# ideafisher/ssUnet-GAN

Hardware: AMD Instinct MI355X
Metric: train images/sec (512^2 tiles) (higher is better)
Workload: dtype f32; 1 GPU; UNet_R_SS_v2 generator + SRGAN-style discriminator, one G+D step (train_seg_gan.py:182-233), 16 x 3x512x512 tiles per GPU, fp32, Adam lr 2e-5; global_batch=16, tile=512, parallelism=dp1, dead_d_param_grads_of_g_step=computed

## Files before the change

ssunet-gan_amd/csrc/conv_wgrad4.hip:

```cpp
#include "common.h"
#include "conv_thin.h"
#include <type_traits>

namespace {

struct W4Args {
  const float* wide; const float* thin; float* ws;
  int Cw, ldw, ldt, N, H, W, Cout, Cin, Cin_real;
  int groups, nz;
  long long units_per_z;
  int segs_per_row;
};

constexpr int SEG = 32;
constexpr int U = 8;

template <bool THIN_COUT, int KS>
__global__ __launch_bounds__(256) void wgrad4_kernel(const W4Args a) {
  constexpr int R = KS / 2, NT = KS * KS, COLS = U + KS - 1;
  const int lane = threadIdx.x & 63;
  const int wave = threadIdx.x >> 6;
  const int zb = blockIdx.x / a.groups, cg = blockIdx.x - zb * a.groups;
  const int z = zb * 4 + wave;
  const int j = lane & 3;
  const int cw = cg * 64 + lane;
  const bool cw_ok = cw < a.Cw;
  const float* tapT = THIN_COUT ? a.wide : a.thin;
  const float* fixT = THIN_COUT ? a.thin : a.wide;
  const unsigned ldtap = THIN_COUT ? a.ldw : a.ldt, ldfix = THIN_COUT ? a.ldt : a.ldw;
  const unsigned npix = (unsigned)(a.N * a.H * a.W);
  const auto tap_rs = __builtin_amdgcn_make_buffer_rsrc(const_cast<float*>(tapT), 0, (int)(npix * ldtap * 4u), 0x00020000);
  const auto fix_rs = __builtin_amdgcn_make_buffer_rsrc(const_cast<float*>(fixT), 0, (int)(npix * ldfix * 4u), 0x00020000);
  const unsigned chtap = THIN_COUT ? cw : j, chfix = THIN_COUT ? j : cw;
  const bool tap_lane_ok = THIN_COUT ? cw_ok : true, fix_lane_ok = THIN_COUT ? true : cw_ok;
  constexpr unsigned OOB = 0xffffffffu;

  f32x4 acc[NT];
#pragma unroll
  for (int t = 0; t < NT; ++t) acc[t] = f32x4{0.f, 0.f, 0.f, 0.f};

  const int u0 = z * (int)a.units_per_z;
  const int total_units = a.N * a.H * a.segs_per_row;
  int u1 = u0 + (int)a.units_per_z; if (u1 > total_units) u1 = total_units;
  for (int u = u0; u < u1; ++u) {
    const int r = u / a.segs_per_row; const int seg = u - r * a.segs_per_row;
    const int y = r % a.H, n = r / a.H;
    const int x0 = seg * SEG;
    const int x1 = x0 + SEG < a.W ? x0 + SEG : a.W;
    unsigned rowoff[KS]; bool rowok[KS];
#pragma unroll
    for (int q = 0; q < KS; ++q) {
      const int iy = y + q - R;
      rowok[q] = tap_lane_ok && (unsigned)iy < (unsigned)a.H;
      rowoff[q] = ((unsigned)((n * a.H + iy) * a.W) * ldtap + chtap) * 4u;
    }
    const unsigned fixoff = ((unsigned)((n * a.H + y) * a.W) * ldfix + chfix) * 4u;
    for (int xb = x0; xb < x1; xb += U) {
      float f[U], v[KS][COLS];
#pragma unroll
      for (int k = 0; k < U; ++k) {
        const bool ok = fix_lane_ok && (xb + k < x1);
        f[k] = __builtin_bit_cast(float, __builtin_amdgcn_raw_buffer_load_b32(
            fix_rs, ok ? fixoff + (unsigned)(xb + k) * ldfix * 4u : OOB, 0, 0));
      }
#pragma unroll
      for (int c = 0; c < COLS; ++c) {
        const int ix = xb + c - R;
        const bool cok = (unsigned)ix < (unsigned)a.W;
        const unsigned xo = (unsigned)ix * ldtap * 4u;
#pragma unroll
        for (int q = 0; q < KS; ++q)
          v[q][c] = __builtin_bit_cast(float, __builtin_amdgcn_raw_buffer_load_b32(
              tap_rs, (cok && rowok[q]) ? rowoff[q] + xo : OOB, 0, 0));
      }
#pragma unroll
      for (int k = 0; k < U; ++k)
#pragma unroll
        for (int q = 0; q < KS; ++q)
#pragma unroll
          for (int e = 0; e < KS; ++e) {
            if (THIN_COUT) acc[q * KS + e] = __builtin_amdgcn_mfma_f32_4x4x1f32(v[q][k + e], f[k], acc[q * KS + e], 0, 0, 0);
            else acc[q * KS + e] = __builtin_amdgcn_mfma_f32_4x4x1f32(f[k], v[q][k + e], acc[q * KS + e], 0, 0, 0);
          }
    }
  }
  __shared__ float red[4][NT * 4][64];
#pragma unroll
  for (int t = 0; t < NT; ++t)
#pragma unroll
    for (int i = 0; i < 4; ++i) red[wave][t * 4 + i][lane] = acc[t][i];
  __syncthreads();
  float* slab = a.ws + (size_t)zb * NT * a.Cin * a.Cout;
  const int b4 = (lane >> 2) * 4;
  for (int e = wave; e < NT * 4; e += 4) {
    const int t = e >> 2, i = e & 3;
    const float sum = ((red[0][e][lane] + red[1][e][lane]) + red[2][e][lane]) + red[3][e][lane];
    int co, c;
    if (THIN_COUT) { co = j; c = cg * 64 + b4 + i; }
    else { co = cg * 64 + b4 + i; c = j; }
    if (co < a.Cout && c < a.Cin) slab[((size_t)t * a.Cin + c) * a.Cout + co] = sum;
  }
}

template <int CR>
__device__ __forceinline__ void wgrad32_cin_body(const W4Args& a, float (*red)[36][64]) {
  const int lane = threadIdx.x & 63, l31 = lane & 31, h = lane >> 5;
  const int wave = threadIdx.x >> 6;
  const int zb = blockIdx.x / a.groups, cg = blockIdx.x - zb * a.groups;
  const int z = zb * 4 + wave;
  const unsigned npix = (unsigned)(a.N * a.H * a.W);
  const auto do_rs = __builtin_amdgcn_make_buffer_rsrc(const_cast<float*>(a.wide), 0, (int)(npix * (unsigned)a.ldw * 4u), 0x00020000);
  const auto in_rs = __builtin_amdgcn_make_buffer_rsrc(const_cast<float*>(a.thin), 0, (int)(npix * (unsigned)a.ldt * 4u), 0x00020000);
  constexpr unsigned OOB = 0xffffffffu;
  const unsigned ldwb = (unsigned)a.ldw * 4u, ldtb = (unsigned)a.ldt * 4u;
  constexpr int NC = CR == 3 ? 27 : 32;
  unsigned aoff[2];
#pragma unroll
  for (int f = 0; f < 2; ++f) { const int co = cg * 64 + f * 32 + l31; aoff[f] = co < a.Cout ? (unsigned)co * 4u : OOB; }
  const int t0 = l31 / CR, c = l31 - t0 * CR;
  const int dy0 = t0 / 3 - 1, dx0 = t0 % 3 - 1;
  const bool col_ok = l31 < NC;

  f32x16 acc[2];
  f32x4 acc8[2];
#pragma unroll
  for (int f = 0; f < 2; ++f) {
#pragma unroll
    for (int q = 0; q < 16; ++q) acc[f][q] = 0.f;
    acc8[f] = f32x4{0.f, 0.f, 0.f, 0.f};
  }

  const int u0 = z * (int)a.units_per_z;
  const int total_units = a.N * a.H * a.segs_per_row;
  int u1 = u0 + (int)a.units_per_z; if (u1 > total_units) u1 = total_units;
  constexpr int UP = 8;
  for (int u = u0; u < u1; ++u) {
    const int r = u / a.segs_per_row; const int seg = u - r * a.segs_per_row;
    const int y = r % a.H, n = r / a.H;
    const int x0 = seg * SEG;
    const int x1 = x0 + SEG < a.W ? x0 + SEG : a.W;
    const unsigned rowpix = (unsigned)((n * a.H + y) * a.W);
    const bool r0ok = col_ok && (unsigned)(y + dy0) < (unsigned)a.H, r8ok = y + 1 < a.H;
    const unsigned b0row = (rowpix + (unsigned)(dy0 * a.W)) * ldtb + (unsigned)c * 4u;
    const unsigned b8row = (rowpix + (unsigned)a.W) * ldtb + (unsigned)(lane & 3) * 4u;
    auto step = [&](auto full_c, const int xb) {
      constexpr bool FULL = decltype(full_c)::value;
      float av[2][UP], bv[UP], b8[UP];
#pragma unroll
      for (int k = 0; k < UP; ++k) {
        const int x = xb + 2 * k + h;
        const bool pok = FULL || x < x1;
        const unsigned po = (rowpix + (unsigned)x) * ldwb;
#pragma unroll
        for (int f = 0; f < 2; ++f)
          av[f][k] = __builtin_bit_cast(float, __builtin_amdgcn_raw_buffer_load_b32(do_rs, (pok && aoff[f] != OOB) ? po + aoff[f] : OOB, 0, 0));
        const int ix0 = x + dx0;
        bv[k] = __builtin_bit_cast(float, __builtin_amdgcn_raw_buffer_load_b32(
            in_rs, (pok && r0ok && (unsigned)ix0 < (unsigned)a.W) ? b0row + (unsigned)ix0 * ldtb : OOB, 0, 0));
        if (CR == 4)
          b8[k] = __builtin_bit_cast(float, __builtin_amdgcn_raw_buffer_load_b32(
              in_rs, (pok && r8ok && x + 1 < a.W) ? b8row + (unsigned)(x + 1) * ldtb : OOB, 0, 0));
      }
#pragma unroll
      for (int k = 0; k < UP; ++k)
#pragma unroll
        for (int f = 0; f < 2; ++f) {
          acc[f] = __builtin_amdgcn_mfma_f32_32x32x2f32(av[f][k], bv[k], acc[f], 0, 0, 0);
          if (CR == 4) acc8[f] = __builtin_amdgcn_mfma_f32_4x4x1f32(av[f][k], b8[k], acc8[f], 0, 0, 0);
        }
    };
    for (int xb = x0; xb < x1; xb += 2 * UP) {
      if (xb + 2 * UP <= x1) step(std::true_type{}, xb);
      else step(std::false_type{}, xb);
    }
  }
  if (col_ok) {
#pragma unroll
    for (int f = 0; f < 2; ++f)
#pragma unroll
      for (int q = 0; q < 16; ++q) red[wave][l31][f * 32 + (q & 3) + 8 * (q >> 2) + 4 * h] = acc[f][q];
  }
  if (CR == 4) {
#pragma unroll
    for (int f = 0; f < 2; ++f)
#pragma unroll
      for (int i = 0; i < 4; ++i) {
        const float odd = __shfl(acc8[f][i], l31 + 32);
        const float s8 = acc8[f][i] + odd;
        if (h == 0) red[wave][32 + (lane & 3)][f * 32 + (l31 & ~3) + i] = s8;
      }
  }
  __syncthreads();
  float* slab = a.ws + (size_t)zb * 9 * a.Cin * a.Cout;
  constexpr int NR = CR == 3 ? 27 : 36;
  for (int e = threadIdx.x; e < NR * 64; e += 256) {
    const int nn = e >> 6, m = e & 63;
    const float sum = ((red[0][nn][m] + red[1][nn][m]) + red[2][nn][m]) + red[3][nn][m];
    const int co = cg * 64 + m;
    const int row = CR == 3 ? nn + nn / 3 : nn;
    if (co < a.Cout) slab[(size_t)row * a.Cout + co] = sum;
  }
}

__global__ __launch_bounds__(256) void wgrad32_cin_kernel(const W4Args a) {
  __shared__ float red[4][36][64];
  if (a.Cin_real == 3) wgrad32_cin_body<3>(a, red);
  else wgrad32_cin_body<4>(a, red);
}

constexpr int TINY_PIX = 4096;

__global__ __launch_bounds__(256) void wgrad_tiny4_kernel(const W4Args a) {
  const int co = threadIdx.x & 7, slot = threadIdx.x >> 3;
  const long long npix = (long long)a.N * a.H * a.W;
  const long long p0 = (long long)blockIdx.x * TINY_PIX;
  const long long p1 = p0 + TINY_PIX < npix ? p0 + TINY_PIX : npix;
  const auto in_rs = __builtin_amdgcn_make_buffer_rsrc(const_cast<float*>(a.thin), 0, (int)((unsigned)npix * (unsigned)a.ldt * 4u), 0x00020000);
  const auto do_rs = __builtin_amdgcn_make_buffer_rsrc(const_cast<float*>(a.wide), 0, (int)((unsigned)npix * (unsigned)a.ldw * 4u), 0x00020000);
  constexpr unsigned OOB = 0xffffffffu;
  const bool co_ok = co < a.Cout;
  f32x4 acc[9];
#pragma unroll
  for (int t = 0; t < 9; ++t) acc[t] = f32x4{0.f, 0.f, 0.f, 0.f};
  for (long long p = p0 + slot; p < p1; p += 32) {
    const int x = (int)(p % a.W); const int y = (int)((p / a.W) % a.H);
    const float g = __builtin_bit_cast(float, __builtin_amdgcn_raw_buffer_load_b32(do_rs, co_ok ? ((unsigned)p * (unsigned)a.ldw + (unsigned)co) * 4u : OOB, 0, 0));
#pragma unroll
    for (int t = 0; t < 9; ++t) {
      const int iy = y + t / 3 - 1, ix = x + t % 3 - 1;
      const bool ok = (unsigned)iy < (unsigned)a.H && (unsigned)ix < (unsigned)a.W;
      const f32x4 v = __builtin_bit_cast(f32x4, __builtin_amdgcn_raw_buffer_load_b128(
          in_rs, ok ? (unsigned)(p + (long long)(t / 3 - 1) * a.W + (t % 3 - 1)) * (unsigned)a.ldt * 4u : OOB, 0, 0));
      acc[t] += v * g;
    }
  }
  __shared__ float red[32][36][8];
#pragma unroll
  for (int t = 0; t < 9; ++t)
#pragma unroll
    for (int c = 0; c < 4; ++c) red[slot][t * 4 + c][co] = acc[t][c];
  __syncthreads();
  float* slab = a.ws + (size_t)blockIdx.x * 9 * a.Cin * a.Cout;
  for (int e = threadIdx.x; e < 36 * 8; e += 256) {
    const int c8 = e & 7, row = e >> 3;
    float sum = 0.f;
#pragma unroll 8
    for (int k = 0; k < 32; ++k) sum += red[k][row][c8];
    const int t = row >> 2, c = row & 3;
    if (c8 < a.Cout && c < a.Cin) slab[((size_t)t * a.Cin + c) * a.Cout + c8] = sum;
  }
}

}

int ssg_wgrad4_kind(const ssg_wgrad_desc* d) {
  if (d->C2 != 0 || d->in_sy != 1 || d->in_sx != 1 || d->GH != d->H || d->GW != d->W) return 0;
  if (d->ntaps == 9) {
    for (int t = 0; t < 9; ++t) if (d->dy[t] != t / 3 - 1 || d->dx[t] != t % 3 - 1) return 0;
  } else if (d->ntaps != 1 || d->dy[0] != 0 || d->dx[0] != 0) {
    return 0;
  }
  if ((long long)d->N * d->H * d->W * (d->ld1 > d->ldd ? d->ld1 : d->ldd) >= (1ll << 30)) return 0;
  if (d->Cout <= 4 && d->C1 >= 16 && d->C1 % 4 == 0) return 5;
  if (d->C1 == 4 && d->Cout <= 8 && d->ntaps == 9) return 7;
  if (d->C1 == 4 && d->ntaps == 9 && d->Cout >= 32 && (long long)d->N * d->H * d->W >= 65536) return 8;
  if (d->C1 == 4) return 6;
  return 0;
}

int ssg_wgrad4_slices(const ssg_wgrad_desc* d, int kind, int* groups, long long* units_per_z, int* segs_per_row) {
  if (kind == 7) {
    if (groups) *groups = 1;
    if (units_per_z) *units_per_z = TINY_PIX;
    if (segs_per_row) *segs_per_row = 1;
    return (int)(((long long)d->N * d->H * d->W + TINY_PIX - 1) / TINY_PIX);
  }
  const int cw = kind == 5 ? d->C1 : d->Cout;
  const int g = (cw + 63) / 64;
  const int spr = (d->W + SEG - 1) / SEG;
  const long long units = (long long)d->N * d->H * spr;
  long long nz = 8192 / g;
  if (nz > units) nz = units;
  if (nz < 1) nz = 1;
  const long long upz = (units + nz - 1) / nz;
  nz = (units + upz - 1) / upz;
  nz = (nz + 3) / 4;
  if (groups) *groups = g;
  if (units_per_z) *units_per_z = upz;
  if (segs_per_row) *segs_per_row = spr;
  return (int)nz;
}

int ssg_wgrad4_launch(const ssg_wgrad_desc* d, int kind, hipStream_t st) {
  W4Args a;
  a.ws = d->ws; a.N = d->N; a.H = d->H; a.W = d->W; a.Cout = d->Cout; a.Cin = d->C1; a.Cin_real = d->Cin_real;
  a.nz = ssg_wgrad4_slices(d, kind, &a.groups, &a.units_per_z, &a.segs_per_row);
  const dim3 grid((unsigned)(a.nz * a.groups)), block(256);
  if (kind == 7) {
    a.wide = d->dout; a.Cw = d->Cout; a.ldw = d->ldd; a.thin = d->in1; a.ldt = d->ld1;
    hipLaunchKernelGGL(wgrad_tiny4_kernel, grid, block, 0, st, a);
    SSG_LAUNCH_CHECK();
    return SSG_OK;
  }
  if (kind == 8) {
    a.wide = d->dout; a.Cw = d->Cout; a.ldw = d->ldd; a.thin = d->in1; a.ldt = d->ld1;
    hipLaunchKernelGGL(wgrad32_cin_kernel, grid, block, 0, st, a);
    SSG_LAUNCH_CHECK();
    return SSG_OK;
  }
  if (kind == 5) { a.wide = d->in1; a.Cw = d->C1; a.ldw = d->ld1; a.thin = d->dout; a.ldt = d->ldd; }
  else { a.wide = d->dout; a.Cw = d->Cout; a.ldw = d->ldd; a.thin = d->in1; a.ldt = d->ld1; }
  if (kind == 5 && d->ntaps == 9) hipLaunchKernelGGL((wgrad4_kernel<true, 3>), grid, block, 0, st, a);
  else if (kind == 5) hipLaunchKernelGGL((wgrad4_kernel<true, 1>), grid, block, 0, st, a);
  else if (d->ntaps == 9) hipLaunchKernelGGL((wgrad4_kernel<false, 3>), grid, block, 0, st, a);
  else hipLaunchKernelGGL((wgrad4_kernel<false, 1>), grid, block, 0, st, a);
  SSG_LAUNCH_CHECK();
  return SSG_OK;
}
```

Before: 92.19 images/sec.

## Add MFMA row-based wgrad kernel for thin-Cout 3x3 weight gradients

Adds a new weight-gradient kernel for thin-output-channel 3x3 convolutions (kind 5). It uses 16x16x4 f32 MFMA instructions over 8-pixel row blocks, with scalar FMA handling the edge taps, and double-buffers the A/B register loads across rows and units. It is dispatched by default when C1 is a multiple of 64 up to 256 and the inputs are 16-byte aligned. The aim is to replace the VALU-bound wgrad4 path with matrix-core throughput, at the cost of complex index and edge logic and higher register pressure.

```diff
diff --git a/ssunet-gan_amd/csrc/conv_wgrad4.hip b/ssunet-gan_amd/csrc/conv_wgrad4.hip
--- a/ssunet-gan_amd/csrc/conv_wgrad4.hip
+++ b/ssunet-gan_amd/csrc/conv_wgrad4.hip
@@ -102,6 +102,149 @@
   }
 }
 
+constexpr int RB = 8;
+constexpr unsigned OOB4 = 0xffffffffu;
+
+struct W4RowsUnit { int n, y, seg, x0, x1, tw; bool ok; };
+struct W4RowsB { f32x4 b[RB], e[2]; };
+struct W4RowsA { float a[RB], e[2][4]; };
+
+__global__ __launch_bounds__(256) __attribute__((amdgpu_waves_per_eu(2))) void wgrad4_rows_kernel(const W4Args a) {
+  const int lane = threadIdx.x & 63, n16 = lane & 15, g = lane >> 4;
+  const int wave = __builtin_amdgcn_readfirstlane(threadIdx.x >> 6);
+  const int zb = blockIdx.x / a.groups, cg = blockIdx.x - zb * a.groups;
+  const int z = zb * 4 + wave;
+  const unsigned npix = (unsigned)(a.N * a.H * a.W);
+  const unsigned ldwb = (unsigned)a.ldw * 4u, ldtb = (unsigned)a.ldt * 4u;
+  const auto d_rs = __builtin_amdgcn_make_buffer_rsrc(const_cast<float*>(a.thin), 0, (int)(npix * ldtb), 0x00020000);
+  const int ea = n16 >> 2, coa = n16 & 3;
+  const bool arow_ok = n16 < 12 && coa < a.Cout;
+  const unsigned xlane = (unsigned)(cg * 64 + 4 * n16) * 4u + (unsigned)(1 + g) * ldwb;
+  const unsigned alane = (unsigned)(2 + g - ea) * ldtb + (unsigned)coa * 4u;
+
+  const int u0 = z * (int)a.units_per_z;
+  const int total_units = a.N * a.H * a.segs_per_row;
+  int u1 = u0 + (int)a.units_per_z; if (u1 > total_units) u1 = total_units;
+
+  auto finish = [&](W4RowsUnit& t, const int u) {
+    t.ok = u < u1;
+    t.x0 = t.seg * SEG;
+    t.x1 = !t.ok ? t.x0 : t.x0 + SEG < a.W ? t.x0 + SEG : a.W;
+    t.tw = (t.x1 - t.x0 + 7) & ~7;
+  };
+  auto first_unit = [&]() {
+    W4RowsUnit t;
+    const int r = u0 / a.segs_per_row;
+    t.seg = u0 - r * a.segs_per_row; t.y = r % a.H; t.n = r / a.H;
+    finish(t, u0);
+    return t;
+  };
+  auto next_unit = [&](const W4RowsUnit& c, const int u) {
+    W4RowsUnit t = c;
+    if (++t.seg == a.segs_per_row) { t.seg = 0; if (++t.y == a.H) { t.y = 0; ++t.n; } }
+    finish(t, u);
+    return t;
+  };
+  auto edge_ix = [&](const W4RowsUnit& t, const int j) {
+    const int T = t.x0 + t.tw;
+    return j == 0 ? (g == 0 ? t.x0 - 1 : g == 1 ? t.x0 : T - 1) : (g == 0 ? t.x0 : g == 1 ? T - 1 : T);
+  };
+  auto load_b = [&](const W4RowsUnit& t, const int q, W4RowsB& B) {
+    const int iy = t.y + q - 1;
+    const bool rok = t.ok && (unsigned)iy < (unsigned)a.H;
+    const auto rs = __builtin_amdgcn_make_buffer_rsrc(const_cast<float*>(a.wide), 0, rok ? (int)(npix * ldwb) : 0, 0x00020000);
+    const unsigned row = (unsigned)((t.n * a.H + iy) * a.W + t.x0) * ldwb;
+    const int lim = (t.tw - 1 < a.W - t.x0 ? t.tw - 1 : a.W - t.x0) - 1;
+#pragma unroll
+    for (int kb = 0; kb < RB; ++kb)
+      B.b[kb] = __builtin_bit_cast(f32x4, __builtin_amdgcn_raw_buffer_load_b128(
+          rs, g < lim - 4 * kb ? xlane + (row + (unsigned)(4 * kb) * ldwb) : OOB4, 0, 0));
+#pragma unroll
+    for (int j = 0; j < 2; ++j) {
+      const int ix = edge_ix(t, j);
+      const bool ok = (g < 3) & ((unsigned)ix < (unsigned)a.W);
+      B.e[j] = __builtin_bit_cast(f32x4, __builtin_amdgcn_raw_buffer_load_b128(
+          rs, ok ? (xlane - (unsigned)(1 + g) * ldwb) + (unsigned)(ix - t.x0) * ldwb + row : OOB4, 0, 0));
+    }
+  };
+  auto load_a = [&](const W4RowsUnit& t, W4RowsA& A) {
+    const unsigned row = (unsigned)((t.n * a.H + t.y) * a.W + t.x0) * ldtb;
+    const int w = t.x1 - t.x0;
+#pragma unroll
+    for (int kb = 0; kb < RB; ++kb) {
+      const bool ok = arow_ok & (g < t.tw - 2 - 4 * kb) & (g - ea < w - 2 - 4 * kb);
+      A.a[kb] = __builtin_bit_cast(float, __builtin_amdgcn_raw_buffer_load_b32(
+          d_rs, ok ? alane + (row + (unsigned)(4 * kb) * ldtb) : OOB4, 0, 0));
+    }
+#pragma unroll
+    for (int j = 0; j < 2; ++j) {
+      const int pw = edge_ix(t, j) - g + 1 - t.x0;
+#pragma unroll
+      for (int r = 0; r < 4; ++r) {
+        const bool ok = (g < 3) & (r < a.Cout) & ((unsigned)pw < (unsigned)w);
+        A.e[j][r] = __builtin_bit_cast(float, __builtin_amdgcn_raw_buffer_load_b32(
+            d_rs, ok ? (unsigned)pw * ldtb + (row + (unsigned)r * 4u) : OOB4, 0, 0));
+      }
+    }
+  };
+
+  f32x4 acc[3][4];
+#pragma unroll
+  for (int q = 0; q < 3; ++q)
+#pragma unroll
+    for (int m = 0; m < 4; ++m) acc[q][m] = f32x4{0.f, 0.f, 0.f, 0.f};
+  auto compute = [&](const int q, const int tw, const W4RowsA& A, const W4RowsB& B) {
+#pragma unroll
+    for (int kb = 0; kb < RB; ++kb) {
+      if (8 * (kb / 2) < tw) {
+#pragma unroll
+        for (int m = 0; m < 4; ++m) acc[q][m] = __builtin_amdgcn_mfma_f32_16x16x4f32(A.a[kb], B.b[kb][m], acc[q][m], 0, 0, 0);
+      }
+    }
+#pragma unroll
+    for (int j = 0; j < 2; ++j)
+#pragma unroll
+      for (int m = 0; m < 4; ++m)
+#pragma unroll
+        for (int r = 0; r < 4; ++r) acc[q][m][r] = __builtin_fmaf(A.e[j][r], B.e[j][m], acc[q][m][r]);
+  };
+
+  W4RowsB B[2]; W4RowsA A[2];
+  W4RowsUnit cur = first_unit();
+  load_a(cur, A[0]); load_b(cur, 0, B[0]);
+  auto unit = [&](auto parity, const int u) {
+    constexpr int P = decltype(parity)::value;
+    const W4RowsUnit nxt = next_unit(cur, u + 1);
+    load_b(cur, 1, B[P ^ 1]);
+    compute(0, cur.tw, A[P], B[P]);
+    load_b(cur, 2, B[P]);
+    compute(1, cur.tw, A[P], B[P ^ 1]);
+    load_a(nxt, A[P ^ 1]); load_b(nxt, 0, B[P ^ 1]);
+    compute(2, cur.tw, A[P], B[P]);
+    cur = nxt;
+  };
+  for (int u = u0; u < u1; u += 2) {
+    unit(std::integral_constant<int, 0>{}, u);
+    if (u + 1 < u1) unit(std::integral_constant<int, 1>{}, u + 1);
+  }
+
+  __shared__ float red[4][48][64];
+#pragma unroll
+  for (int q = 0; q < 3; ++q)
+#pragma unroll
+    for (int m = 0; m < 4; ++m)
+#pragma unroll
+      for (int r = 0; r < 4; ++r) red[wave][(q * 4 + m) * 4 + r][lane] = acc[q][m][r];
+  __syncthreads();
+  float* slab = a.ws + (size_t)zb * 9 * a.Cin * a.Cout;
+  for (int i = wave; i < 48; i += 4) {
+    const int q = i >> 4, m = (i >> 2) & 3, co = i & 3;
+    const float sum = ((red[0][i][lane] + red[1][i][lane]) + red[2][i][lane]) + red[3][i][lane];
+    const int c = cg * 64 + 4 * n16 + m;
+    if (g < 3 && co < a.Cout && c < a.Cin) slab[((size_t)(q * 3 + g) * a.Cin + c) * a.Cout + co] = sum;
+  }
+}
+
 template <int CR>
 __device__ __forceinline__ void wgrad32_cin_body(const W4Args& a, float (*red)[36][64]) {
   const int lane = threadIdx.x & 63, l31 = lane & 31, h = lane >> 5;
@@ -291,6 +434,18 @@
   return (int)nz;
 }
 
+static int g_rows_mode = 1;
+static bool wgrad4_rows_ok(const ssg_wgrad_desc* d, int kind) {
+  return g_rows_mode && kind == 5 && d->ntaps == 9 && d->C1 % 64 == 0 && d->C1 <= 256 && d->ld1 % 4 == 0 && ((uintptr_t)d->in1 & 15) == 0;
+}
+
+extern "C" int ssg_wgrad4_body(const ssg_wgrad_desc* d) {
+  if (!d) return 0;
+  const int kind = ssg_wgrad4_kind(d);
+  return kind != 5 ? 0 : wgrad4_rows_ok(d, kind) ? 2 : 1;
+}
+extern "C" int ssg_wgrad4_rows_mode(int on) { const int was = g_rows_mode; g_rows_mode = on ? 1 : 0; return was; }
+
 int ssg_wgrad4_launch(const ssg_wgrad_desc* d, int kind, hipStream_t st) {
   W4Args a;
   a.ws = d->ws; a.N = d->N; a.H = d->H; a.W = d->W; a.Cout = d->Cout; a.Cin = d->C1; a.Cin_real = d->Cin_real;
@@ -310,7 +465,8 @@
   }
   if (kind == 5) { a.wide = d->in1; a.Cw = d->C1; a.ldw = d->ld1; a.thin = d->dout; a.ldt = d->ldd; }
   else { a.wide = d->dout; a.Cw = d->Cout; a.ldw = d->ldd; a.thin = d->in1; a.ldt = d->ld1; }
-  if (kind == 5 && d->ntaps == 9) hipLaunchKernelGGL((wgrad4_kernel<true, 3>), grid, block, 0, st, a);
+  if (wgrad4_rows_ok(d, kind)) hipLaunchKernelGGL(wgrad4_rows_kernel, grid, block, 0, st, a);
+  else if (kind == 5 && d->ntaps == 9) hipLaunchKernelGGL((wgrad4_kernel<true, 3>), grid, block, 0, st, a);
   else if (kind == 5) hipLaunchKernelGGL((wgrad4_kernel<true, 1>), grid, block, 0, st, a);
   else if (d->ntaps == 9) hipLaunchKernelGGL((wgrad4_kernel<false, 3>), grid, block, 0, st, a);
   else hipLaunchKernelGGL((wgrad4_kernel<false, 1>), grid, block, 0, st, a);
```

New measurement: 92.07 images/sec. No clear change (-0.1%).
